# YamaguchiAtsushi/pointcloud_processor

Measured on AMD Instinct MI355X. Metric: ray-hit tests/sec + candidate poses/sec (whole node), 1M-pt terrain, higher is better.
Workload: dtype f64 march / f32 point test; 1 GPU; C2: 1M-pt L-shape excavation terrain, 1024x256 ray fan, 256 candidate poses per GPU; terrain_points=1001740, poses_total=256, num_candidates_lattice=348, parallelism=pose-shard x1

## Files before the change

pointcloud_processor_amd/_stamps.py:

```python
from __future__ import annotations

import hashlib
import os
from pathlib import Path

ROOT = Path(__file__).resolve().parents[1]
CSRC = ROOT / "pointcloud_processor_amd" / "csrc"
_COMMON = ["pcp_internal.hpp", "pcp_knobs.hpp", "Makefile", "../../include/pcp_abi.h"]
WORKLOAD_SOURCES = {
    "fan": ["pcp_fan.hip", "pcp_march.hpp", "pcp_fine.hip", "pcp_index.hip", "pcp_stencil.hpp",
            "pcp_grid.hpp", "pcp_fan_band.hpp", "pcp_fan_clear.hpp", "pcp_fan_clip.hpp",
            "pcp_fan_pivot.hpp", "pcp_fan_row.hpp"] + _COMMON,
    "filter": ["pcp_filter.hip", "pcp_rigid.hpp"] + _COMMON,
    "cells": ["pcp_score.hip", "pcp_march.hpp", "pcp_fine.hip", "pcp_index.hip", "pcp_stencil.hpp",
              "pcp_grid.hpp", "pcp_fan_band.hpp", "pcp_fan_clear.hpp", "pcp_fan_clip.hpp",
              "pcp_fan_pivot.hpp", "pcp_fan_row.hpp"] + _COMMON,
}


def workload_stamp(key: str) -> str:
    h = hashlib.sha256(os.environ.get("EXTRA", "").encode())
    for name in WORKLOAD_SOURCES[key]:
        f = (CSRC / name).resolve()
        h.update(name.encode())
        h.update(f.read_bytes())
    return h.hexdigest()[:16]
```

pointcloud_processor_amd/csrc/pcp_fan.hip:

```cpp
#pragma clang fp contract(off)

#include <algorithm>
#include <cmath>
#include <cstring>
#include <vector>

#include <hip/hip_ext.h>

#include "pcp_fan_cull.hpp"
#include "pcp_fan_dir.hpp"
#include "pcp_internal.hpp"
#include "pcp_march.hpp"

namespace pcp {

struct FanArgs {
    GridView g;
    const double *ca, *sa, *ce, *se;
    const double *pose;
    const double *steps;
    int K;
    int n_az;
    int uniform_el;
    uint32_t rays;
    uint32_t waves;
    float r2, rexit;
    int present;
    int16_t *first_hit;
    uint32_t w0, lw;
    int rev;
    uint2 *wave_part;
    uint32_t P;
    unsigned long long *stats;
};

enum { FAN_PLAIN = (int)FanMode::Plain, FAN_STATS = (int)FanMode::Stats,
       FAN_STAMPS = (int)FanMode::Stamps };

__device__ __forceinline__ uint32_t wave_sum_u32(uint32_t v) {
    v += (uint32_t)__builtin_amdgcn_update_dpp(0, (int)v, 0x128, 0xF, 0xF, false);
    v += (uint32_t)__builtin_amdgcn_update_dpp(0, (int)v, 0x124, 0xF, 0xF, false);
    v += (uint32_t)__builtin_amdgcn_update_dpp(0, (int)v, 0x122, 0xF, 0xF, false);
    v += (uint32_t)__builtin_amdgcn_update_dpp(0, (int)v, 0x121, 0xF, 0xF, false);
    return (uint32_t)__builtin_amdgcn_readlane((int)v, 0) +
           (uint32_t)__builtin_amdgcn_readlane((int)v, 16) +
           (uint32_t)__builtin_amdgcn_readlane((int)v, 32) +
           (uint32_t)__builtin_amdgcn_readlane((int)v, 48);
}

template <int MODE, int BS, bool ZB = true, int FN = 0, bool UE = false, int NPW = 1,
          bool SL = false, bool MT = false, bool SP = false>
__device__ __forceinline__ void fan_body(const FanArgs &a, uint32_t p0, uint32_t rblock) {
    static_assert(!MT || MODE == FAN_PLAIN, "the mounted march has no diagnostic modes");
    static_assert(!SP || !MT, "the mounted kernels keep the run-time layout tests");
    constexpr int PR = MT ? kFanDirRow : kFanRow;
    static_assert(PR * 32 * sizeof(double) + kStepLds * sizeof(double) <= 160 * 1024 / 8,
                  "at the widest NPW at least 8 one-wave workgroups per CU keep their LDS");
    const uint32_t ray = rblock * BS + threadIdx.x;
    const uint32_t wid = ray >> 6;
    const bool active = ray < a.rays;
    double lx = 0.0, ly = 0.0, lz = 0.0;
    __shared__ double s_steps[SL ? kStepLds : 1];
    __shared__ double s_pose[SL ? PR * NPW : 1];
    if (SL) {
        for (int q = threadIdx.x; q < a.K; q += BS) s_steps[q] = a.steps[q];
        for (int q = threadIdx.x; q < PR * NPW; q += BS) s_pose[q] = a.pose[PR * (size_t)p0 + q];
        __syncthreads();
    }
    const double *steps = SL ? s_steps : a.steps;
    uint32_t ju = 0;
    if (UE)
        ju = (uint32_t)__builtin_amdgcn_readfirstlane(
            (int)((rblock * BS + (threadIdx.x & ~63u)) / (uint32_t)a.n_az));
    if (active && a.present) {
        const uint32_t j = UE ? (rblock * BS + (threadIdx.x & ~63u)) / (uint32_t)a.n_az
                              : ray / (uint32_t)a.n_az;
        const uint32_t i = ray - j * (uint32_t)a.n_az;
        const double cej = a.ce[j];
        lx = cej * a.ca[i];
        ly = cej * a.sa[i];
        lz = a.se[j];
    }
#pragma unroll 1
    for (int q = 0; q < NPW; ++q) {
    const uint32_t p = p0 + (uint32_t)q;
    const uint32_t wslot = p * a.waves + wid;
    unsigned long long t0 = 0, t1 = 0, t2 = 0;
    if (MODE == FAN_STAMPS) t0 = __builtin_amdgcn_s_memtime();
    int hit = -1;
    uint32_t cnt[4] = {0, 0, 0, 0};
    const double *P = SL ? s_pose + PR * q : a.pose + PR * (size_t)p;
    bool dead = false;
    FanDir md{0.0, 0.0, 0.0};
    if (MT) md = fan_dir(P, lx, ly, lz);
    if (UE && !MT) {
        const uint2 lr = *reinterpret_cast<const uint2 *>(P + FR_LIVE);
        const uint32_t j0 = (uint32_t)__builtin_amdgcn_readfirstlane((int)lr.x);
        const uint32_t j1 = (uint32_t)__builtin_amdgcn_readfirstlane((int)lr.y);
        dead = ju < j0 || ju >= j1;
        if (MODE == FAN_STAMPS && dead) t1 = t0;
    }
    if (!dead && active && a.present) {
        const double cy = MT ? 0.0 : P[FR_CY], sy = MT ? 0.0 : P[FR_SY];
        const double dx = MT ? md.x : cy * lx - sy * ly;
        const double dy = MT ? md.y : sy * lx + cy * ly;
        const double dz = MT ? md.z : lz;
        if (MODE == FAN_STAMPS) {
            asm volatile("" ::"v"(dx), "v"(dy));
            t1 = __builtin_amdgcn_s_memtime();
        }
#ifdef PCP_FAN_NO_ROW
        constexpr bool ROW = false;
#else
        constexpr bool ROW = !MT;
#endif
        hit = march<MODE == FAN_STATS, ZB, 1, FN, true, true, ROW, SP>(
            a.g, P[0], P[1], P[2], dx, dy, dz, steps, a.K, 1e300, a.r2, a.rexit, cnt, 0, 1,
            MT ? nullptr : fan_row_floats(P));
    }
    if (MODE == FAN_STAMPS) {
        asm volatile("" ::"v"(hit));
        t2 = __builtin_amdgcn_s_memtime();
    }
    if (active && a.first_hit) a.first_hit[(size_t)p * a.rays + ray] = (int16_t)hit;
    uint2 part;
    if (UE && !MT && dead) {
        part = make_uint2(0u, 64u * (uint32_t)a.K);
    } else {
        const uint64_t bal = __ballot(active && hit >= 0);
        uint32_t u = active ? (hit >= 0 ? (uint32_t)hit + 1u : (uint32_t)a.K) : 0u;
        part = make_uint2((uint32_t)__popcll(bal), wave_sum_u32(u));
    }
    if ((threadIdx.x & 63) == 0 && wid < a.waves) {
        a.wave_part[(size_t)p * a.lw + (wid - a.w0)] = part;
    }
    if (MODE == FAN_STATS) {
        const size_t nw = (size_t)a.P * a.waves;
#pragma unroll
        for (int c = 0; c < 4; ++c) {
            unsigned long long v = c < 3 ? cnt[c] : (FN ? cnt[3] : cnt[1]);
#pragma unroll
            for (int o = 32; o > 0; o >>= 1) v += __shfl_xor(v, o, 64);
            if ((threadIdx.x & 63) == 0 && wid < a.waves) a.stats[c * nw + wslot] = v;
        }
    }
    if (MODE == FAN_STAMPS && (threadIdx.x & 63) == 0 && wid < a.waves) {
        const unsigned long long t3 = __builtin_amdgcn_s_memtime();
        unsigned long long *o = a.stats + 4 * (size_t)wslot;
        o[0] = t0;
        o[1] = t1;
        o[2] = t2;
        o[3] = t3;
    }
    }
}

template <int MODE, int BS = 64, bool ZB = true, int W = 7, int FN = 0, bool UE = false,
          bool MT = false>
__global__ void __launch_bounds__(BS) __attribute__((amdgpu_waves_per_eu(W, W)))
k_raycast_fan(FanArgs a, uint32_t P) {
    fan_body<MODE, BS, ZB, FN, UE, 1, false, MT>(a, blockIdx.x % P, a.w0 + blockIdx.x / P);
}

template <int MODE, int BS = 64, bool ZB = true, int W = 8, int FN = 1, bool UE = true, int NPW = 1,
          bool MT = false, bool SP = false>
__global__ void __launch_bounds__(BS) __attribute__((amdgpu_waves_per_eu(W, W)))
k_raycast_fan_xcd(FanArgs a, uint32_t P) {
    const uint32_t pc = P >> 3, gpc = pc / NPW, j = blockIdx.x >> 3;
    const uint32_t b = j / gpc;
    fan_body<MODE, BS, ZB, FN, UE, NPW, true, MT, SP>(a, (blockIdx.x & 7u) * pc + (j % gpc) * NPW,
                                                      a.w0 + (a.rev ? a.lw - 1u - b : b));
}

template <int BS, bool ZB>
__global__ void __launch_bounds__(BS) __attribute__((amdgpu_waves_per_eu(7, 7)))
k_raycast_fan_pm(FanArgs a, uint32_t) {
    fan_body<FAN_PLAIN, BS, ZB>(a, blockIdx.y, blockIdx.x);
}

__global__ void __launch_bounds__(1024)
k_sum_u64(const unsigned long long *__restrict__ in, size_t n, unsigned long long *__restrict__ out) {
    const unsigned long long *row = in + (size_t)blockIdx.x * n;
    unsigned long long v = 0;
    for (size_t k = threadIdx.x; k < n; k += 1024) v += row[k];
#pragma unroll
    for (int o = 32; o > 0; o >>= 1) v += __shfl_xor(v, o, 64);
    __shared__ unsigned long long sw[16];
    if ((threadIdx.x & 63) == 0) sw[threadIdx.x >> 6] = v;
    __syncthreads();
    if (threadIdx.x == 0) {
        unsigned long long t = 0;
        for (int w = 0; w < 16; ++w) t += sw[w];
        out[blockIdx.x] = t;
    }
}

__global__ void __launch_bounds__(kT)
k_fan_reduce(const uint2 *__restrict__ part, uint32_t waves,
             uint32_t *__restrict__ blocked, unsigned long long *__restrict__ units,
             unsigned long long *__restrict__ keys, uint32_t lo, uint32_t Pall,
             unsigned long long units_culled, int16_t *__restrict__ fh, uint32_t rays,
             uint32_t r_lo, uint32_t r_hi) {
    const uint32_t p = blockIdx.x;
    if (fh) {
        int16_t *row = fh + (size_t)p * rays;
        for (uint32_t r = threadIdx.x; r < r_lo; r += kT) row[r] = (int16_t)-1;
        for (uint32_t r = r_hi + threadIdx.x; r < rays; r += kT) row[r] = (int16_t)-1;
    }
    if (keys)
        for (uint32_t i = p * kT + threadIdx.x; i <= Pall; i += gridDim.x * kT)
            if (i < lo || i - lo >= gridDim.x) keys[i] = ~0ull;
    const uint2 *row = part + (size_t)p * waves;
    uint32_t b = 0;
    unsigned long long u = 0;
    for (uint32_t w = threadIdx.x; w < waves; w += kT) {
        const uint2 v = row[w];
        b += v.x;
        u += v.y;
    }
#pragma unroll
    for (int o = 32; o > 0; o >>= 1) {
        b += __shfl_xor(b, o, 64);
        u += __shfl_xor(u, o, 64);
    }
    __shared__ uint32_t sb[kT / 64];
    __shared__ unsigned long long su[kT / 64];
    if ((threadIdx.x & 63) == 0) {
// ... 430 lines not shown
```

pointcloud_processor_amd/csrc/pcp_fine.hip:

```cpp
#pragma clang fp contract(off)

#include <cfloat>
#include <cmath>

#include <rocprim/device/device_radix_sort.hpp>

#include "pcp_fan_band.hpp"
#include "pcp_fan_clear.hpp"
#include "pcp_fan_pivot.hpp"
#include "pcp_grid.hpp"
#include "pcp_internal.hpp"

namespace pcp {

namespace {

constexpr int kThreads = 256;

struct FineGeo {
    double ox, oy;
    double cf, inv_cf;
    double R2;
    int32_t fnx, fny;
    int32_t reach;
};

__device__ __forceinline__ bool in_window(const FineGeo &f, double px, double py, int wx, int wy) {
    const double x0 = f.ox + (double)wx * f.cf, y0 = f.oy + (double)wy * f.cf;
    const double dx = fmax(fmax(x0 - px, px - (x0 + f.cf)), 0.0);
    const double dy = fmax(fmax(y0 - py, py - (y0 + f.cf)), 0.0);
    return dx * dx + dy * dy <= f.R2;
}

__device__ __forceinline__ void fine_cell(const FineGeo &f, float x, float y, int &cx, int &cy) {
    cx = min(max((int)floor(((double)x - f.ox) * f.inv_cf), 0), f.fnx - 1);
    cy = min(max((int)floor(((double)y - f.oy) * f.inv_cf), 0), f.fny - 1);
}

__global__ void __launch_bounds__(kThreads)
k_zkeys(const float4 *__restrict__ pts, uint32_t n, unsigned long long *__restrict__ key,
        uint32_t *__restrict__ val) {
    const uint32_t i = blockIdx.x * kThreads + threadIdx.x;
    if (i >= n) return;
    const float4 p = pts[i];
    uint32_t u = __float_as_uint(p.z);
    u = (u & 0x80000000u) ? ~u : (u | 0x80000000u);
    key[i] = ((unsigned long long)(~u) << 32) | __float_as_uint(p.w);
    val[i] = i;
}

__global__ void __launch_bounds__(kThreads)
k_win_count(const float4 *__restrict__ pts, const uint32_t *__restrict__ zord, uint32_t n,
            FineGeo f, uint32_t *__restrict__ pcount) {
    const uint32_t i = blockIdx.x * kThreads + threadIdx.x;
    if (i >= n) return;
    const float4 p = pts[zord[i]];
    int cx, cy;
    fine_cell(f, p.x, p.y, cx, cy);
    uint32_t c = 0;
    for (int wy = max(cy - f.reach, 0); wy <= min(cy + f.reach, f.fny - 1); ++wy)
        for (int wx = max(cx - f.reach, 0); wx <= min(cx + f.reach, f.fnx - 1); ++wx)
            if (in_window(f, (double)p.x, (double)p.y, wx, wy)) ++c;
    pcount[i] = c;
}

__global__ void __launch_bounds__(kThreads)
k_win_emit(const float4 *__restrict__ pts, const uint32_t *__restrict__ zord, uint32_t n,
           FineGeo f, const uint32_t *__restrict__ poff, uint32_t *__restrict__ wkey,
           uint32_t *__restrict__ rank) {
    const uint32_t i = blockIdx.x * kThreads + threadIdx.x;
    if (i >= n) return;
    const float4 p = pts[zord[i]];
    int cx, cy;
    fine_cell(f, p.x, p.y, cx, cy);
    uint32_t o = poff[i];
    for (int wy = max(cy - f.reach, 0); wy <= min(cy + f.reach, f.fny - 1); ++wy)
        for (int wx = max(cx - f.reach, 0); wx <= min(cx + f.reach, f.fnx - 1); ++wx)
            if (in_window(f, (double)p.x, (double)p.y, wx, wy)) {
                wkey[o] = (uint32_t)wx + (uint32_t)f.fnx * (uint32_t)wy;
                rank[o] = i;
                ++o;
            }
}

__global__ void __launch_bounds__(kThreads)
k_win_bounds(const uint32_t *__restrict__ wkey, uint32_t np, uint32_t nw,
             uint32_t *__restrict__ cstart) {
    const uint32_t w = blockIdx.x * kThreads + threadIdx.x;
    if (w > nw) return;
    uint32_t lo = 0, hi = np;
    while (lo < hi) {
        const uint32_t mid = (lo + hi) >> 1;
        if (wkey[mid] < w) lo = mid + 1;
        else hi = mid;
    }
    cstart[w] = lo;
}

__global__ void __launch_bounds__(kThreads)
k_win_place(const float4 *__restrict__ pts, const uint32_t *__restrict__ zord,
            const uint32_t *__restrict__ wkey, const uint32_t *__restrict__ rank, uint32_t np,
            float4 *__restrict__ wpts) {
    const uint32_t k = blockIdx.x * kThreads + threadIdx.x;
    if (k >= np) return;
    wpts[k + wkey[k]] = pts[zord[rank[k]]];
}

__global__ void __launch_bounds__(kThreads)
k_frec(float4 *__restrict__ wpts, const uint32_t *__restrict__ cstart, CellMap m, double c,
       uint32_t fnx, uint32_t fny, uint32_t rz, uint32_t tsteps, int tile,
       int skip2, uint2 *__restrict__ frec, uint16_t *__restrict__ fband,
       uint32_t *__restrict__ fstart) {
    const uint32_t nw = fnx * fny, w = blockIdx.x * kThreads + threadIdx.x;
    const uint32_t sh = tile == 2 ? 3u : 2u, T = 1u << sh, TS = T * T;
    const uint32_t tx = (fnx + T - 1) >> sh, ty = (fny + T - 1) >> sh;
    const size_t plane = tile ? (size_t)tx * ty * TS : (size_t)nw;
    auto put = [&](size_t r, uint32_t start, uint32_t band) {
        if (tile == 2) {
            fband[r] = (uint16_t)band;
            fstart[r] = start;
        } else {
            frec[r] = make_uint2(start, band);
        }
    };
    if (tile && w < tx * ty * TS) {
        const uint32_t t = w >> (2 * sh), sub = w & (TS - 1);
        const uint32_t px = (t % tx) * T + (sub & (T - 1)), py = (t / tx) * T + (sub >> sh);
        if (px >= fnx || py >= fny)
            for (uint32_t iz = 0; iz < rz; ++iz) put((size_t)iz * plane + w, 0u, 0x00FFu);
    }
    if (w >= nw) return;
    const uint32_t wx = w % fnx, wy = w / fnx;
    const size_t base = tile ? ((size_t)((wy >> sh) * tx + (wx >> sh)) << (2 * sh)) |
                                   ((wy & (T - 1)) << sh) | (wx & (T - 1))
                             : (size_t)w;
    const uint32_t s = cstart[w] + w, e = cstart[w + 1] + w;
    wpts[e] = make_float4(__int_as_float(0x7FC00000), __int_as_float(0x7FC00000), -INFINITY,
                          __uint_as_float(0xFFFFFFFFu));
    uint32_t jt = s, jb = s, j2 = s, j3 = s;
    float zt = wpts[s].z, zb = zt, zlast = zt, z2 = zt, z3 = zt;
    int ct = s < e ? cell_z(m, zt) : -1, cb = ct;
    for (int iz = (int)rz - 1; iz >= 0; --iz) {
        while (jt < e && ct > iz + 1) {
            ++jt;
            zt = wpts[jt].z;
            ct = jt < e ? cell_z(m, zt) : -1;
        }
        if (jb < jt) {
            jb = jt;
            zb = zt;
            cb = ct;
        }
        while (jb < e && cb >= iz) {
            zlast = zb;
            ++jb;
            zb = wpts[jb].z;
            cb = jb < e ? cell_z(m, zb) : -1;
        }
        uint32_t band = 0x00FFu;
        if (jb > jt) {
            const uint32_t code = zband_code(zt, zlast, m.oz + (double)iz * c, c);
            const uint32_t lo = code & 255u, hi = code >> 8;
            const uint32_t lo2 = (lo == 0u || lo <= tsteps) ? 0u : lo - tsteps;
            const uint32_t hi2 = (hi == 255u) ? 255u : min(hi + tsteps, 255u);
// ... 113 lines not shown
}

__global__ void __launch_bounds__(kThreads)
k_pivot(const float4 *__restrict__ wpts, const uint32_t *__restrict__ cstart, FineGeo f,
        uint32_t tx, uint32_t nslot, float *__restrict__ piv) {
    const uint32_t t = blockIdx.x * kThreads + threadIdx.x;
    if (t >= nslot) return;
    const uint32_t tile = t >> 6, sub = t & 63u;
    const uint32_t wx = (tile % tx) * 8u + (sub & 7u), wy = (tile / tx) * 8u + (sub >> 3);
    float3 best = make_float3(__int_as_float(0x7FC00000), __int_as_float(0x7FC00000), -INFINITY);
    if (wx < (uint32_t)f.fnx && wy < (uint32_t)f.fny) {
        const uint32_t w = wx + (uint32_t)f.fnx * wy;
        const uint32_t s = cstart[w] + w, e = cstart[w + 1] + w;
        PivotKey kb{};
        for (uint32_t j = s; j < e; ++j) {
            const float4 p = wpts[j];
            const PivotKey k{pivot_d2(f.ox, f.oy, f.cf, wx, wy, p.x, p.y), p.z,
                             __float_as_uint(p.w)};
            if (j == s || pivot_better(k, kb)) {
                kb = k;
                best = make_float3(p.x, p.y, p.z);
            }
        }
    }
    float *o = piv + 3 * (size_t)t;
    o[0] = best.x;
    o[1] = best.y;
    o[2] = best.z;
}

__global__ void __launch_bounds__(kThreads)
k_pack3(const float4 *__restrict__ src, uint32_t n, float *__restrict__ dst) {
    const uint32_t i = blockIdx.x * kThreads + threadIdx.x;
    if (i >= n) return;
    const float4 p = src[i];
    dst[3 * (size_t)i] = p.x;
    dst[3 * (size_t)i + 1] = p.y;
    dst[3 * (size_t)i + 2] = p.z;
}

struct FinePlan {
    CellMap m;
    FineGeo f;
    ClearGeo cg;
    int F, tile;
    uint64_t fnx, fny, rz, nw, nrec;
    uint64_t npiv;
    size_t band_bytes, rec_bytes;
    uint32_t tsteps;
};

FinePlan fine_plan(const GridIndex &g, int F, int tile) {
    FinePlan p{};
    const GridView gv = g.view();
    p.m = CellMap{gv.ox, gv.oy, gv.oz, gv.inv_c, g.nx, g.ny, g.nz};
    p.F = F;
    p.tile = tile;
    p.fnx = (uint64_t)F * g.nx;
    p.fny = (uint64_t)F * g.ny;
    p.rz = (uint64_t)(g.nz > 1 ? g.nz - 1 : 0);
    const uint64_t T = tile == 2 ? 8 : 4;
    p.nrec = tile ? ((p.fnx + T - 1) / T) * ((p.fny + T - 1) / T) * T * T * p.rz
                  : p.fnx * p.fny * p.rz;
    p.nw = p.fnx * p.fny;
    p.npiv = tile == 2 ? (uint64_t)pivot_tiles((uint32_t)p.fnx) * pivot_tiles((uint32_t)p.fny) * 64
                       : 0;
    p.band_bytes = ((size_t)p.nrec * 2 + 255) & ~(size_t)255;
    p.rec_bytes = tile == 2 ? p.band_bytes + (size_t)p.nrec * 4 : (size_t)p.nrec * sizeof(uint2);
    p.f.ox = gv.ox;
    p.f.oy = gv.oy;
    p.f.cf = g.c / F;
    p.f.inv_cf = F * gv.inv_c;
    const double R = g.r_q + kQueryMargin;
    p.f.R2 = R * R;
    p.f.fnx = (int32_t)p.fnx;
    p.f.fny = (int32_t)p.fny;
    p.f.reach = (int32_t)std::ceil(R / p.f.cf);
    p.tsteps = (uint32_t)std::ceil((g.r_q + 2e-3) / g.c / (double)kZq);
    const double zabs = std::fmax(std::fabs(gv.oz), std::fabs(gv.oz + (double)g.nz * g.c));
    p.cg = fan_clear_geo(gv.oz, g.c, R, zabs);
    return p;
}

}

int build_fine(pcp_ctx *ctx, GridIndex &g) {
    if (g.fine_ok || g.fine_fail || !g.present || !g.occz_ok || g.n_pts == 0) return PCP_OK;
    hipStream_t st = ctx->stream;
    ProfScope prof(ctx, PCP_K_INDEX_BUILD);
    const FinePlan plan = fine_plan(g, std::max(2, std::min(ctx->knob.terrain_fine, 8)),
                                    ctx->knob.fine_tile == 2 ? 2 : ctx->knob.fine_tile ? 1 : 0);
    const CellMap m = plan.m;
    const FineGeo f = plan.f;
    const int F = plan.F, tile = plan.tile;
    const uint64_t fnx = plan.fnx, fny = plan.fny, rz = plan.rz, nrec = plan.nrec, nw = plan.nw;
    const size_t band_bytes = plan.band_bytes, rec_bytes = plan.rec_bytes;
    if (rz == 0 || nrec >= (1ull << 29) || fnx >= (1ull << 24) || fny * rz >= (1ull << 24)) {
        g.fine_fail = true;
        return PCP_OK;
    }
    const uint32_t n = (uint32_t)g.n_pts;
    const unsigned gridn = (n + kThreads - 1) / kThreads;
    const float4 *pts = g.pts.as<const float4>();
    size_t t1 = 0, t2 = 0;
    (void)rocprim::radix_sort_pairs(nullptr, t1, (unsigned long long *)nullptr,
                                    (unsigned long long *)nullptr, (uint32_t *)nullptr,
                                    (uint32_t *)nullptr, n, 0u, 64u, st);
    PCP_HIP(ctx, ctx->scratch[2].ensure((size_t)n * 24 + 64));
    unsigned long long *k0 = ctx->scratch[2].as<unsigned long long>(), *k1 = k0 + n;
    uint32_t *v0 = reinterpret_cast<uint32_t *>(k1 + n), *zord = v0 + n;
    hipLaunchKernelGGL(k_zkeys, dim3(gridn), dim3(kThreads), 0, st, pts, n, k0, v0);
    PCP_CHECK_LAUNCH(ctx);
    PCP_HIP(ctx, ctx->scratch[3].ensure((size_t)(n + 1) * 8 + (nw + 1) * 4 + 64));
    uint32_t *pcount = ctx->scratch[3].as<uint32_t>(), *poff = pcount + (n + 1);
    uint32_t *cstart = poff + (n + 1);
    const size_t tscan = scan_tmp_bytes(std::max<uint64_t>(n, nw)) +
                         (std::max<uint64_t>(n, nw) + 1) * sizeof(uint32_t);
    PCP_HIP(ctx, ctx->scratch[4].ensure(std::max(t1, tscan) + 256));
    if (rocprim::radix_sort_pairs(ctx->scratch[4].p, t1, k0, k1, v0, zord, n, 0u, 64u, st) !=
        hipSuccess)
        return set_err(ctx, PCP_E_HIP, "build_fine: z sort failed");
    hipLaunchKernelGGL(k_win_count, dim3(gridn), dim3(kThreads), 0, st, pts, zord, n, f, pcount);
    PCP_CHECK_LAUNCH(ctx);
    int rc = exclusive_scan_u32(ctx, pcount, poff, n, ctx->scratch[4].p);
    if (rc) return rc;
    uint32_t np = 0;
    if ((rc = read_small(ctx, &np, poff + n, 4, st))) return rc;
    if (np == 0 || (uint64_t)np + nw >= (1ull << 28)) {
        g.fine_fail = true;
        return PCP_OK;
    }
    int wbits = 1;
    while ((1ull << wbits) < nw) ++wbits;
    (void)rocprim::radix_sort_pairs(nullptr, t2, (uint32_t *)nullptr, (uint32_t *)nullptr,
                                    (uint32_t *)nullptr, (uint32_t *)nullptr, np, 0u,
                                    (unsigned)wbits, st);
    PCP_HIP(ctx, ctx->scratch[5].ensure((size_t)np * 16 + 64));
    uint32_t *wk0 = ctx->scratch[5].as<uint32_t>(), *wk1 = wk0 + np, *rk0 = wk1 + np,
             *rk1 = rk0 + np;
    PCP_HIP(ctx, ctx->scratch[6].ensure(t2 + 256));
    hipLaunchKernelGGL(k_win_emit, dim3(gridn), dim3(kThreads), 0, st, pts, zord, n, f,
                       (const uint32_t *)poff, wk0, rk0);
    PCP_CHECK_LAUNCH(ctx);
    if (rocprim::radix_sort_pairs(ctx->scratch[6].p, t2, wk0, wk1, rk0, rk1, np, 0u,
                                  (unsigned)wbits, st) != hipSuccess)
        return set_err(ctx, PCP_E_HIP, "build_fine: window sort failed");
    hipLaunchKernelGGL(k_win_bounds, dim3((unsigned)((nw + kThreads) / kThreads)), dim3(kThreads),
                       0, st, (const uint32_t *)wk1, np, (uint32_t)nw, cstart);
    PCP_CHECK_LAUNCH(ctx);
    const size_t nent = (size_t)np + nw;
    const bool pack = ctx->knob.fine_pack != 0;
    const bool pivots = tile == 2 && plan.npiv < (1ull << 28);
    if ((pack && ctx->scratch[7].ensure(nent * sizeof(float4)) != hipSuccess) ||
        g.wpts.ensure(pack ? nent * 12 + 16 : nent * sizeof(float4)) != hipSuccess ||
        g.frec.ensure(rec_bytes) != hipSuccess ||
        (pivots && g.fpiv.ensure(plan.npiv * kPivotBytes + 16) != hipSuccess)) {
        (void)hipGetLastError();
        g.wpts.release();
        g.frec.release();
        g.fpiv.release();
        g.fine_fail = true;
        return PCP_OK;
    }
    float4 *went = pack ? ctx->scratch[7].as<float4>() : g.wpts.as<float4>();
    hipLaunchKernelGGL(k_win_place, dim3((np + kThreads - 1) / kThreads), dim3(kThreads), 0, st,
                       pts, (const uint32_t *)zord, (const uint32_t *)wk1, (const uint32_t *)rk1,
                       np, went);
    PCP_CHECK_LAUNCH(ctx);
    const bool skip2 = tile == 2 && ctx->knob.fine_skip == 2 && nent < (1ull << 25);
    const uint32_t tsteps = plan.tsteps;
    const uint64_t nthr = std::max<uint64_t>(nw, tile ? nrec / rz : 0);
    hipLaunchKernelGGL(k_frec, dim3((unsigned)((nthr + kThreads - 1) / kThreads)), dim3(kThreads), 0,
                       st, went, (const uint32_t *)cstart, m, g.c, (uint32_t)fnx,
                       (uint32_t)fny, (uint32_t)rz, tsteps, tile, skip2 ? 1 : 0,
                       g.frec.as<uint2>(),
                       g.frec.as<uint16_t>(),
                       reinterpret_cast<uint32_t *>(g.frec.as<char>() + band_bytes));
    PCP_CHECK_LAUNCH(ctx);
    if (pivots) {
        hipLaunchKernelGGL(k_pivot, dim3((unsigned)((plan.npiv + kThreads - 1) / kThreads)),
                           dim3(kThreads), 0, st, (const float4 *)went, (const uint32_t *)cstart,
                           f, pivot_tiles((uint32_t)fnx), (uint32_t)plan.npiv,
                           g.fpiv.as<float>());
        PCP_CHECK_LAUNCH(ctx);
    }
    if (tile == 2) {
        const size_t lev_bytes = ((size_t)nw * 4 + 255) & ~(size_t)255;
        PCP_HIP(ctx, ctx->scratch[5].ensure(lev_bytes + (size_t)nw * rz * 2 + 64));
        uint32_t *lev = ctx->scratch[5].as<uint32_t>();
        uint16_t *hcol = reinterpret_cast<uint16_t *>(ctx->scratch[5].as<char>() + lev_bytes);
        const ClearGeo cg = plan.cg;
        PCP_HIP(ctx, hipMemsetAsync(lev, 0xFF, (size_t)nw * 4, st));
        hipLaunchKernelGGL(k_clear_level, dim3(gridn), dim3(kThreads), 0, st, pts, n, f, cg,
                           (int)rz, lev);
        PCP_CHECK_LAUNCH(ctx);
        const dim3 cgrid((unsigned)((nw + kThreads - 1) / kThreads), (unsigned)rz);
        hipLaunchKernelGGL(k_clear_col, dim3(cgrid.x), dim3(kThreads), 0, st,
                           (const uint32_t *)lev, (int)fnx, (int)fny, (uint32_t)nw, (uint32_t)rz,
                           hcol);
        PCP_CHECK_LAUNCH(ctx);
        hipLaunchKernelGGL(k_clear_code, cgrid, dim3(kThreads), 0, st, (const uint16_t *)hcol,
                           (int)fnx, (int)fny, (uint32_t)nw, (uint32_t)((fnx + 7) / 8), (size_t)(nrec / rz),
                           g.frec.as<uint16_t>());
        PCP_CHECK_LAUNCH(ctx);
        g.fband_ok = false;
        if (g.fband2.ensure(band_bytes) == hipSuccess) {
            PCP_HIP(ctx, hipMemcpyAsync(g.fband2.p, g.frec.p, band_bytes, hipMemcpyDeviceToDevice,
                                        st));
            hipLaunchKernelGGL(k_band_tight, dim3(cgrid.x), dim3(kThreads), 0, st,
                               (const float4 *)went, (const uint32_t *)cstart, m, f, g.c,
                               kQueryMargin, g.r_q + kBandMu, (uint32_t)rz,
                               (uint32_t)((fnx + 7) / 8), (size_t)(nrec / rz),
                               g.frec.as<const uint16_t>(), g.fband2.as<uint16_t>());
            PCP_CHECK_LAUNCH(ctx);
            g.fband_ok = true;
        } else {
            (void)hipGetLastError();
            g.fband2.release();
        }
    }
    if (pack) {
        hipLaunchKernelGGL(k_pack3, dim3((unsigned)((nent + kThreads - 1) / kThreads)),
                           dim3(kThreads), 0, st, (const float4 *)went, (uint32_t)nent,
                           g.wpts.as<float>());
        PCP_CHECK_LAUNCH(ctx);
    }
    g.wpack = pack ? 1 : 0;
    g.frx = (uint32_t)fnx;
    g.fry = (uint32_t)fny;
    g.frz = (uint32_t)rz;
    g.ffine = (float)F;
    g.ftile = tile;
    g.fskip = skip2 ? 2 : 1;
    g.fstart_off = tile == 2 ? band_bytes : 0;
    g.fnent = nent;
    g.fpiv_ok = pivots;
    g.fine_ok = true;
    return PCP_OK;
}

}

extern "C" int pcp_debug_fine_copy(pcp_ctx *ctx, pcp_fine_geo *geo, void *frec,
                                   uint64_t frec_cap, void *wpts, uint64_t wpts_cap, void *pts,
                                   uint64_t pts_cap) {
    using namespace pcp;
    if (!ctx || !geo) return PCP_E_INVALID;
    const GridIndex &g = ctx->terrain;
    *geo = pcp_fine_geo{};
    if (!g.present || !g.fine_ok) return PCP_OK;
    const FinePlan p = fine_plan(g, (int)g.ffine, g.ftile);
    geo->built = 1;
    geo->tile = g.ftile;
    geo->skip = g.fskip;
    geo->packed = g.wpack;
    geo->nx = g.nx;
    geo->ny = g.ny;
    geo->nz = g.nz;
    geo->F = p.F;
    geo->reach = p.f.reach;
    geo->fnx = p.f.fnx;
    geo->fny = p.f.fny;
    geo->rz = (int32_t)p.rz;
    geo->tsteps = (int32_t)p.tsteps;
    geo->n_points = g.n_pts;
    geo->n_records = p.nrec;
    geo->n_entries = g.fnent;
    geo->start_off = g.fstart_off;
    geo->frec_bytes = p.rec_bytes;
    geo->wpts_bytes = g.fnent * (g.wpack ? 12u : 16u);
    geo->pts_bytes = g.n_pts * sizeof(float4);
    geo->ox = p.m.ox;
    geo->oy = p.m.oy;
    geo->oz = p.m.oz;
    geo->c = g.c;
    geo->inv_c = p.m.inv_c;
    geo->r_q = g.r_q;
    geo->cf = p.f.cf;
    geo->inv_cf = p.f.inv_cf;
    geo->R2 = p.f.R2;
    geo->zq = (double)kZq;
    geo->clear_zt0 = p.cg.zt0;
    geo->clear_c = p.cg.c;
    if (!frec && !wpts && !pts) return PCP_OK;
    if ((frec && frec_cap < geo->frec_bytes) || (wpts && wpts_cap < geo->wpts_bytes) ||
        (pts && pts_cap < geo->pts_bytes))
        return set_err(ctx, PCP_E_CAPACITY, "pcp_debug_fine_copy: a buffer is too small");
    PCP_HIP(ctx, hipSetDevice(ctx->device));
    PCP_HIP(ctx, hipStreamSynchronize(ctx->stream));
    if (frec) PCP_HIP(ctx, hipMemcpy(frec, g.frec.p, geo->frec_bytes, hipMemcpyDeviceToHost));
    if (wpts) PCP_HIP(ctx, hipMemcpy(wpts, g.wpts.p, geo->wpts_bytes, hipMemcpyDeviceToHost));
    if (pts) PCP_HIP(ctx, hipMemcpy(pts, g.pts.p, geo->pts_bytes, hipMemcpyDeviceToHost));
    return PCP_OK;
}

extern "C" int pcp_debug_fine_pivot(pcp_ctx *ctx, pcp_fine_pivot_geo *geo, void *piv,
                                    uint64_t piv_cap) {
    using namespace pcp;
    if (!ctx || !geo) return PCP_E_INVALID;
    const GridIndex &g = ctx->terrain;
    *geo = pcp_fine_pivot_geo{};
    if (!g.present || !g.fine_ok || !g.fpiv_ok) return PCP_OK;
    const FinePlan p = fine_plan(g, (int)g.ffine, g.ftile);
    geo->built = 1;
    geo->enabled = ctx->knob.fan_pivot ? 1 : 0;
    geo->fnx = p.f.fnx;
    geo->fny = p.f.fny;
// ... 35 lines not shown
```

pointcloud_processor_amd/csrc/pcp_march.hpp:

```cpp
#pragma once

#include <cfloat>

#include "pcp_fan_clear.hpp"
#include "pcp_fan_clip.hpp"
#include "pcp_fan_row.hpp"
#include "pcp_internal.hpp"
#include "pcp_stencil.hpp"

namespace pcp {

constexpr int kT = 256;
#ifndef PCP_CELL_PROBES
#define PCP_CELL_PROBES 1
#endif

__device__ __forceinline__ bool stencil_cell(const GridView &g, float qx, float qy, float qz,
                                             uint32_t &lin) {
    uint32_t ix, iy, iz;
    const bool ok = stencil_cell3_fb(g, qx, qy, qz, ix, iy, iz);
    lin = ix + (uint32_t)g.nx * (iy + (uint32_t)g.ny * iz);
    return ok;
}

template <bool STATS>
__device__ __forceinline__ bool scan_stencil(const GridView &g, uint32_t lin, float qx, float qy,
                                             float qz, float r2, uint32_t *cnt) {
    const uint32_t nx = (uint32_t)g.nx, nxy = nx * (uint32_t)g.ny;
    uint32_t b[4][3];
#pragma unroll
    for (int r = 0; r < 4; ++r) {
        const U3 u = ld_u3o(g.start, lin + (r & 1) * nx + (r >> 1) * nxy);
        b[r][0] = u.a;
        b[r][1] = u.b;
        b[r][2] = u.c;
    }
    P3 f[8];
#pragma unroll
    for (int i = 0; i < 8; ++i) {
        const uint32_t k = b[i >> 1][i & 1];
        f[i] = ld_p3o(g.pts, k < b[i >> 1][(i & 1) + 1] ? k : 0u);
    }
    uint32_t live = 0;
#pragma unroll
    for (int i = 0; i < 8; ++i) {
        const uint32_t k = b[i >> 1][i & 1], e = b[i >> 1][(i & 1) + 1];
        if (k < e) {
            if (STATS) cnt[2] += 1;
            if (flann_within(qx, qy, qz, f[i], r2)) return true;
            const float dz = qz - f[i].z;
            if (!(dz >= 0.0f && dz * dz >= r2) && k + 1 < e) live |= 1u << i;
        }
    }
    if (!live) return false;
#pragma unroll
    for (int i = 0; i < 8; ++i) {
        if (!(live & (1u << i))) continue;
        const uint32_t e = b[i >> 1][(i & 1) + 1];
        for (uint32_t k = b[i >> 1][i & 1] + 1; k < e; k += 2) {
            const P3 p0 = ld_p3o(g.pts, k);
            const P3 p1 = ld_p3o(g.pts, min(k + 1, e - 1));
            if (STATS) cnt[2] += 1;
            if (flann_within(qx, qy, qz, p0, r2)) return true;
            float dz = qz - p0.z;
            if (dz >= 0.0f && dz * dz >= r2) break;
            if (k + 1 >= e) break;
            if (STATS) cnt[2] += 1;
            if (flann_within(qx, qy, qz, p1, r2)) return true;
            dz = qz - p1.z;
            if (dz >= 0.0f && dz * dz >= r2) break;
        }
    }
    return false;
}

#ifndef PCP_BLK_STEP
#define PCP_BLK_STEP 1
#endif
__device__ __forceinline__ uint32_t mad_u24(uint32_t a, uint32_t b, uint32_t c) {
    uint32_t d;
    asm("v_mad_u32_u24 %0, %1, %2, %3" : "=v"(d) : "v"(a), "v"(b), "v"(c));
    return d;
}
template <class T>
__device__ __forceinline__ T vgpr_pin(T x) {
#ifndef PCP_NO_VGPR_PIN
    asm("" : "+v"(x));
#endif
    return x;
}

template <bool STATS>
__device__ __forceinline__ bool scan_run(const float4 *pts, uint32_t k0, uint32_t e, float qx,
                                         float qy, float qz, float r2, uint32_t *cnt) {
    for (uint32_t k = k0; k < e; k += PCP_BLK_STEP) {
        P3 p[PCP_BLK_STEP];
#pragma unroll
        for (int i = 0; i < PCP_BLK_STEP; ++i) p[i] = ld_p3o(pts, min(k + i, e - 1));
#pragma unroll
        for (int i = 0; i < PCP_BLK_STEP; ++i) {
            if (i > 0 && k + i >= e) return false;
            if (STATS) cnt[2] += 1;
            if (flann_within(qx, qy, qz, p[i], r2)) return true;
            const float dz = qz - p[i].z;
            if (dz >= 0.0f && dz * dz >= r2) return false;
        }
    }
    return false;
}

template <bool STATS>
__device__ __forceinline__ bool scan_window3(const float *pts, uint32_t k, float qx, float qy,
                                             float qz, float r2, float rexit, uint32_t *cnt) {
    bool within, stop;
    do {
        const float *f = reinterpret_cast<const float *>(reinterpret_cast<const char *>(pts) +
                                                         ((k << 3) + (k << 2)));
        const P3 p = P3{f[0], f[1], f[2]};
        ++k;
        if (STATS) cnt[2] += 1;
#ifdef PCP_WALK_CENSUS
        if (STATS && p.z - qz >= rexit) cnt[3] += 1;
#endif
        within = flann_within(qx, qy, qz, p, r2);
        stop = within | (qz - p.z >= rexit);
    } while (!stop);
    return within;
}

template <bool STATS>
__device__ __forceinline__ bool scan_window(const float4 *pts, uint32_t k, float qx, float qy,
                                            float qz, float r2, float rexit, uint32_t *cnt) {
    bool within, stop;
    do {
        const P3 p = ld_p3o(pts, k++);
        if (STATS) cnt[2] += 1;
#ifdef PCP_WALK_CENSUS
        if (STATS && p.z - qz >= rexit) cnt[3] += 1;
#endif
        within = flann_within(qx, qy, qz, p, r2);
        stop = within | (qz - p.z >= rexit);
    } while (!stop);
    return within;
}

template <bool STATS>
__device__ __forceinline__ bool scan_block(const GridView &g, uint32_t lin, float qx, float qy,
                                           float qz, float r2, uint32_t *cnt) {
    const uint2 se = ld_u2o(g.bstart, lin);
    return scan_run<STATS>(g.bpts, se.x, se.y, qx, qy, qz, r2, cnt);
}

template <bool STATS>
__device__ __forceinline__ bool scan_corner(const GridView &g, uint32_t lin, float qx, float qy,
                                            float qz, float r2, uint32_t *cnt) {
    if (g.bpts) return scan_block<STATS>(g, lin, qx, qy, qz, r2, cnt);
    return scan_stencil<STATS>(g, lin, qx, qy, qz, r2, cnt);
}

__device__ __forceinline__ bool stencil_any(const GridView &g, float qx, float qy, float qz,
                                            float r2) {
    uint32_t lin;
    if (!stencil_cell(g, qx, qy, qz, lin)) return false;
    if (!((ld_u32o(g.occ2, lin >> 5) >> (lin & 31)) & 1u)) return false;
    return scan_stencil<false>(g, lin, qx, qy, qz, r2, nullptr);
}

__device__ __forceinline__ void clip_kf(const GridView &g, double px, double py, double pz,
                                        double dx, double dy, double dz, int K, int &klo,
                                        int &khi) {
    const float p[3] = {(float)px, (float)py, (float)pz};
    const float inv[3] = {__builtin_amdgcn_rcpf((float)dx), __builtin_amdgcn_rcpf((float)dy),
                          __builtin_amdgcn_rcpf((float)dz)};
    fan_clip(g.fb, p, inv, (float)(1.0 / kRayStep), g.fclip_e, K, klo, khi);
}
__device__ __forceinline__ void clip_kf_row(const GridView &g, const float *rel, double dx,
                                            double dy, double dz, int K, int &klo, int &khi) {
    const float inv[3] = {__builtin_amdgcn_rcpf((float)dx), __builtin_amdgcn_rcpf((float)dy),
                          __builtin_amdgcn_rcpf((float)dz)};
    fan_clip_rel(rel, inv, (float)(1.0 / kRayStep), g.fclip_e, K, klo, khi);
}

template <bool STATS, bool ZB = true, int NB = 1, int FN = 0, bool CLR = false, bool PIV = false,
          bool ROW = false, bool SP = false>
__device__ __forceinline__ int march(const GridView &g, double px, double py, double pz,
                                     double dx, double dy, double dz,
                                     const double *__restrict__ steps, int K, double end,
                                     float r2, float rexit, uint32_t *cnt = nullptr,
                                     int koff = 0, int kstr = 1, const float *rowf = nullptr) {
    static_assert(!SP || FN == 8, "the layout facts are the split records'");
    if (FN == 2) {
        if (g.frec && g.ftile == 2)
            return march<STATS, ZB, NB, 8, CLR, PIV, ROW>(g, px, py, pz, dx, dy, dz, steps, K,
                                                          end, r2, rexit, cnt, koff, kstr, rowf);
        if (g.frec && g.ftile)
            return march<STATS, ZB, NB, 4, CLR, PIV, ROW>(g, px, py, pz, dx, dy, dz, steps, K,
                                                          end, r2, rexit, cnt, koff, kstr, rowf);
        if (g.frec)
            return march<STATS, ZB, NB, 1, CLR, PIV, ROW>(g, px, py, pz, dx, dy, dz, steps, K,
                                                          end, r2, rexit, cnt, koff, kstr, rowf);
        return march<STATS, ZB, NB, 0, CLR, PIV, ROW>(g, px, py, pz, dx, dy, dz, steps, K, end,
                                                      r2, rexit, cnt, koff, kstr, rowf);
    }
    int klo, khi;
    if (ROW) clip_kf_row(g, rowf + FRF_CLIP, dx, dy, dz, K, klo, khi);
    else clip_kf(g, px, py, pz, dx, dy, dz, K, klo, khi);
    if (end < 1e299) {
        const double ke = floor((end - 0.5) / kRayStep) + 1.0;
        khi = (int)fmin((double)khi, fmax(ke, -1.0));
    }
    if (klo > khi) return -1;
    const float fdx = (float)dx, fdy = (float)dy, fdz = (float)dz;
    const float sc = (float)kRayStep * g.finv_c, h = 0.5f * g.finv_c;
    const float Dx = fdx * sc, Dy = fdy * sc, Dz = fdz * sc;
    const float Ax = (ROW ? rowf[FRF_BASE] : ((float)px - g.flo_x) * g.finv_c) + fdx * h;
    const float Ay = (ROW ? rowf[FRF_BASE + 1] : ((float)py - g.flo_y) * g.finv_c) + fdy * h;
    const float Az = (ROW ? rowf[FRF_BASE + 2] : ((float)pz - g.flo_z) * g.finv_c) + fdz * h;
    const uint32_t nx = (uint32_t)g.nx, ny = (uint32_t)g.ny;
    if (FN == 1 || FN == 4 || FN == 8) {
        const float F = g.ffine;
        const float D2x = F * Dx, D2y = F * Dy, A2x = F * (Ax + g.fzoff), A2y = F * (Ay + g.fzoff);
        const uint32_t mx = g.frx - 1, my = g.fry - 1, mz = g.frz - 1;
        const float fmx = (float)mx, fmy = (float)my, fmz = (float)mz;
        (void)mx, (void)my, (void)mz, (void)fmx, (void)fmy, (void)fmz;
        const uint32_t rxs = FN == 4 ? (g.frx + 3) >> 2 : FN == 8 ? (g.frx + 7) >> 3 : g.frx;
        const uint32_t rys = FN == 4 ? (g.fry + 3) >> 2 : FN == 8 ? (g.fry + 7) >> 3 : g.fry;
        const uint32_t rx = FN == 8 ? vgpr_pin(rxs) : rxs, ry = FN == 8 ? vgpr_pin(rys) : rys;
        const float fus_off = FN == 8 ? vgpr_pin(g.fus_off) : g.fus_off;
        const ClearRay cr = FN == 8 && CLR ? fan_clear_ray(fdx, fdy, fdz, (float)kRayStep, g.fclr_cf,
                                                    g.fclr_rb, SP || g.fclear != 0)
                                    : ClearRay{0.0f, 0.0f};
        for (int k = klo + koff, jump = 0; k <= khi; k += kstr * (1 + jump / kstr)) {
            const float kf = (float)k;
            const float fx = __builtin_fmaf(D2x, kf, A2x);
            const float fy = __builtin_fmaf(D2y, kf, A2y);
            const float fz = __builtin_fmaf(Dz, kf, Az);
#ifdef PCP_CLAMP_INT
            const uint32_t ix = min((uint32_t)fmaxf(fx, 0.0f), mx);
            const uint32_t iy = min((uint32_t)fmaxf(fy, 0.0f), my);
            const uint32_t iz = min((uint32_t)fmaxf(fz, 0.0f), mz);
#else
            const uint32_t ix = (uint32_t)__builtin_amdgcn_fmed3f(fx, 0.0f, fmx);
            const uint32_t iy = (uint32_t)__builtin_amdgcn_fmed3f(fy, 0.0f, fmy);
            const uint32_t iz = (uint32_t)__builtin_amdgcn_fmed3f(fz, 0.0f, fmz);
#endif
            const uint32_t ri = FN == 8 ? (mad_u24(rx, mad_u24(ry, iz, iy >> 3), ix >> 3) << 6) |
                                              ((iy & 7u) << 3) | (ix & 7u)
                              : FN == 4 ? (mad_u24(rx, mad_u24(ry, iz, iy >> 2), ix >> 2) << 4) |
                                              ((iy & 3u) << 2) | (ix & 3u)
                                        : mad_u24(rx, mad_u24(ry, iz, iy), ix);
            uint2 R = make_uint2(0u, 0u);
            if (FN == 8) R.y = ld_u16o(g.fband, ri);
            else R = ld_rec(g.frec, ri);
            const float us = __builtin_fmaf(fz - (float)iz, 1.0f / kZq, fus_off);
            const float lo = (float)(R.y & 255u);
            const bool cand = (us < (float)((R.y >> 8) & 255u)) & (us > lo);
            jump = (FN == 8 && CLR && lo == 255.0f) ? fan_clear_skip((float)(R.y >> 8), cr)
                                                    : 0;
            if (FN == 8 && CLR) asm volatile("" : "+v"(jump));
            if (STATS) cnt[0] += 1;
            if (cand) {
                const double s = steps[k];
                if (!(s < end)) return -1;
                const float qx = (float)(px + dx * s);
                const float qy = (float)(py + dy * s);
                const float qz = (float)(pz + dz * s);
                if (FN == 8 && PIV && (SP || g.fpiv)) {
                    const uint32_t pi = (mad_u24(rx, iy >> 3, ix >> 3) << 6) | (ri & 63u);
                    const float *pf = reinterpret_cast<const float *>(
                        reinterpret_cast<const char *>(g.fpiv) + ((pi << 3) + (pi << 2)));
                    const P3 pv = P3{pf[0], pf[1], pf[2]};
                    if (STATS) cnt[2] += 1;
                    if (flann_within(qx, qy, qz, pv, r2)) return k;
                }
                if (STATS) cnt[1] += 1;
                uint32_t w0 = R.x;
                if (FN == 8) {
                    const uint32_t ws = ld_u32o(g.fstart, ri);
                    if (SP || g.fskip == 2) {
                        const float ha = __builtin_fmaf((float)iz + 1.375f, g.fzc, g.fzo);
                        const float hb = __builtin_fmaf((float)iz + 1.6875f, g.fzc, g.fzo);
                        const float marg = 1e-4f + 4.0f * FLT_EPSILON *
                                                       (fmaxf(fabsf(ha), fabsf(hb)) +
                                                        fabsf(g.fzo) + fabsf(qz));
                        const float v = qz + (rexit + marg);
                        w0 = (ws & 0x01FFFFFFu) +
                             (v < ha ? (ws >> 25) & 15u : v < hb ? ws >> 29 : 0u);
                    } else {
                        const float h2 = __builtin_fmaf((float)iz + 1.5f, g.fzc, g.fzo);
                        const float marg =
                            1e-4f + 4.0f * FLT_EPSILON * (fabsf(h2) + fabsf(g.fzo) + fabsf(qz));
                        w0 = (ws & 0x0FFFFFFFu) + (qz + (rexit + marg) < h2 ? ws >> 28 : 0u);
                    }
                }
                const bool packed = SP || g.wpack;
                if (packed ? scan_window3<STATS>(reinterpret_cast<const float *>(g.wpts), w0, qx,
                                                 qy, qz, r2, rexit, cnt)
                           : scan_window<STATS>(g.wpts, w0, qx, qy, qz, r2, rexit, cnt))
                    return k;
            }
        }
        return -1;
    }
    if (NB > 1 && ZB) {
        for (int k0 = klo + NB * koff; k0 <= khi; k0 += NB * kstr) {
            uint32_t zz[NB], izs[NB];
            float fzs[NB];
#pragma unroll
            for (int b = 0; b < NB; ++b) {
                const float kf = (float)(k0 + b);
                const float fx = __builtin_fmaf(Dx, kf, Ax);
                const float fy = __builtin_fmaf(Dy, kf, Ay);
                const float fz = __builtin_fmaf(Dz, kf, Az);
                const bool ok = (k0 + b <= khi) & (fx >= 0.0f) & (fx < g.fnx1) & (fy >= 0.0f) &
                                (fy < g.fny1) & (fz >= 0.0f) & (fz < g.fnz1);
                const uint32_t izc = ok ? (uint32_t)fz : 0u;
                const uint32_t lin = ok ? (uint32_t)fx + nx * ((uint32_t)fy + ny * izc) : 0u;
                zz[b] = ok ? ld_u16o(g.occz, lin) : 0x00FFu;
                izs[b] = izc;
                fzs[b] = fz;
            }
#pragma unroll
            for (int b = 0; b < NB; ++b) {
                const int k = k0 + b;
                const uint32_t lo = zz[b] & 255u, hi = zz[b] >> 8;
                const float u = fzs[b] - (float)izs[b] + g.fzoff;
                const bool cand = (lo <= hi) & ((hi == 255u) | (u - (float)hi * kZq < g.fzt)) &
                                  ((lo == 0u) | ((float)lo * kZq - u < g.fzt));
                if (STATS && k <= khi) cnt[0] += 1;
                if (cand) {
                    const double s = steps[k];
                    if (!(s < end)) return -1;
                    if (STATS) cnt[1] += 1;
                    const float qx = (float)(px + dx * s);
                    const float qy = (float)(py + dy * s);
                    const float qz = (float)(pz + dz * s);
                    uint32_t l2;
                    if (stencil_cell(g, qx, qy, qz, l2) && scan_corner<STATS>(g, l2, qx, qy, qz, r2, cnt))
                        return k;
                }
            }
        }
        return -1;
    }
    for (int k = klo + koff; k <= khi; k += kstr) {
        const float kf = (float)k;
        const float fx = __builtin_fmaf(Dx, kf, Ax);
        const float fy = __builtin_fmaf(Dy, kf, Ay);
        const float fz = __builtin_fmaf(Dz, kf, Az);
        const bool ok = (fx >= 0.0f) & (fx < g.fnx1) & (fy >= 0.0f) & (fy < g.fny1) &
                        (fz >= 0.0f) & (fz < g.fnz1);
        const uint32_t izc = ok ? (uint32_t)fz : 0u;
        const uint32_t lin = ok ? (uint32_t)fx + nx * ((uint32_t)fy + ny * izc) : 0u;
        bool cand;
        if (ZB) {
            const uint32_t zz = ok ? ld_u16o(g.occz, lin) : 0x00FFu;
            const uint32_t lo = zz & 255u, hi = zz >> 8;
            const float u = fz - (float)izc + g.fzoff;
            cand = (lo <= hi) & ((hi == 255u) | (u - (float)hi * kZq < g.fzt)) &
                   ((lo == 0u) | ((float)lo * kZq - u < g.fzt));
        } else {
            const uint32_t word = ok ? ld_u32o(g.occ2, lin >> 5) : 0u;
            cand = (word >> (lin & 31u)) & 1u;
        }
        if (STATS) cnt[0] += 1;
        if (cand) {
            const double s = steps[k];
            if (!(s < end)) return -1;
            if (STATS) cnt[1] += 1;
            const float qx = (float)(px + dx * s);
            const float qy = (float)(py + dy * s);
            const float qz = (float)(pz + dz * s);
            uint32_t l2;
            if (stencil_cell(g, qx, qy, qz, l2) && scan_corner<STATS>(g, l2, qx, qy, qz, r2, cnt))
                return k;
        }
    }
    return -1;
}

}
```

Before: 8028 billion ray-hit tests/s.

## Pair-unroll packed window walk and hoist fan prologue loads before barrier

The packed 12-byte window scan now loads two consecutive entries per trip and tests them in order, so each iteration issues both loads up front instead of serialising one load per test. The allocation grows by a slack entry so the speculative second read stays in bounds. Separately, the shared-memory prologue now loads the step table, pose rows and trig values into registers before writing LDS and hitting the barrier, which lets all global loads overlap. The cost is extra loads on walks that stop after the first entry, plus more registers.

```diff
diff --git a/pointcloud_processor_amd/_stamps.py b/pointcloud_processor_amd/_stamps.py
--- a/pointcloud_processor_amd/_stamps.py
+++ b/pointcloud_processor_amd/_stamps.py
@@ -10,11 +10,11 @@
 WORKLOAD_SOURCES = {
     "fan": ["pcp_fan.hip", "pcp_march.hpp", "pcp_fine.hip", "pcp_index.hip", "pcp_stencil.hpp",
             "pcp_grid.hpp", "pcp_fan_band.hpp", "pcp_fan_clear.hpp", "pcp_fan_clip.hpp",
-            "pcp_fan_pivot.hpp", "pcp_fan_row.hpp"] + _COMMON,
+            "pcp_fan_pivot.hpp", "pcp_fan_row.hpp", "pcp_walk_pair.hpp"] + _COMMON,
     "filter": ["pcp_filter.hip", "pcp_rigid.hpp"] + _COMMON,
     "cells": ["pcp_score.hip", "pcp_march.hpp", "pcp_fine.hip", "pcp_index.hip", "pcp_stencil.hpp",
               "pcp_grid.hpp", "pcp_fan_band.hpp", "pcp_fan_clear.hpp", "pcp_fan_clip.hpp",
-              "pcp_fan_pivot.hpp", "pcp_fan_row.hpp"] + _COMMON,
+              "pcp_fan_pivot.hpp", "pcp_fan_row.hpp", "pcp_walk_pair.hpp"] + _COMMON,
 }
 
 
diff --git a/pointcloud_processor_amd/csrc/pcp_fan.hip b/pointcloud_processor_amd/csrc/pcp_fan.hip
--- a/pointcloud_processor_amd/csrc/pcp_fan.hip
+++ b/pointcloud_processor_amd/csrc/pcp_fan.hip
@@ -61,8 +61,46 @@
     const bool active = ray < a.rays;
     double lx = 0.0, ly = 0.0, lz = 0.0;
     __shared__ double s_steps[SL ? kStepLds : 1];
-    __shared__ double s_pose[SL ? PR * NPW : 1];
-    if (SL) {
+    __shared__ double s_pose[SL ? (PR * NPW + BS - 1) / BS * BS : 1];
+#ifdef PCP_FAN_NO_PRO1
+    constexpr bool PRO1 = false;
+#else
+    constexpr bool PRO1 = SL;
+#endif
+    if (PRO1) {
+        constexpr int NS = kStepLds / BS, NR = (PR * NPW + BS - 1) / BS;
+        static_assert(kStepLds % BS == 0, "whole trips over the step table");
+        double sv[NS], rv[NR], cej = 0.0, cai = 0.0, sai = 0.0, sej = 0.0;
+#pragma unroll
+        for (int t = 0; t < NS; ++t) {
+            const int q = (int)threadIdx.x + t * BS;
+            sv[t] = q < a.K ? a.steps[q] : 0.0;
+        }
+#pragma unroll
+        for (int t = 0; t < NR; ++t) {
+            const int q = (int)threadIdx.x + t * BS;
+            rv[t] = q < PR * NPW ? a.pose[PR * (size_t)p0 + q] : 0.0;
+        }
+        if (active && a.present) {
+            const uint32_t j = UE ? (rblock * BS + (threadIdx.x & ~63u)) / (uint32_t)a.n_az
+                                  : ray / (uint32_t)a.n_az;
+            const uint32_t i = ray - j * (uint32_t)a.n_az;
+            cej = a.ce[j];
+            cai = a.ca[i];
+            sai = a.sa[i];
+            sej = a.se[j];
+        }
+#pragma unroll
+        for (int t = 0; t < NS; ++t) s_steps[threadIdx.x + t * BS] = sv[t];
+#pragma unroll
+        for (int t = 0; t < NR; ++t) s_pose[threadIdx.x + t * BS] = rv[t];
+        __syncthreads();
+        if (active && a.present) {
+            lx = cej * cai;
+            ly = cej * sai;
+            lz = sej;
+        }
+    } else if (SL) {
         for (int q = threadIdx.x; q < a.K; q += BS) s_steps[q] = a.steps[q];
         for (int q = threadIdx.x; q < PR * NPW; q += BS) s_pose[q] = a.pose[PR * (size_t)p0 + q];
         __syncthreads();
@@ -72,7 +110,7 @@
     if (UE)
         ju = (uint32_t)__builtin_amdgcn_readfirstlane(
             (int)((rblock * BS + (threadIdx.x & ~63u)) / (uint32_t)a.n_az));
-    if (active && a.present) {
+    if (!PRO1 && active && a.present) {
         const uint32_t j = UE ? (rblock * BS + (threadIdx.x & ~63u)) / (uint32_t)a.n_az
                               : ray / (uint32_t)a.n_az;
         const uint32_t i = ray - j * (uint32_t)a.n_az;
diff --git a/pointcloud_processor_amd/csrc/pcp_fine.hip b/pointcloud_processor_amd/csrc/pcp_fine.hip
--- a/pointcloud_processor_amd/csrc/pcp_fine.hip
+++ b/pointcloud_processor_amd/csrc/pcp_fine.hip
@@ -10,6 +10,7 @@
 #include "pcp_fan_pivot.hpp"
 #include "pcp_grid.hpp"
 #include "pcp_internal.hpp"
+#include "pcp_walk_pair.hpp"
 
 namespace pcp {
 
@@ -429,7 +430,8 @@
     const bool pack = ctx->knob.fine_pack != 0;
     const bool pivots = tile == 2 && plan.npiv < (1ull << 28);
     if ((pack && ctx->scratch[7].ensure(nent * sizeof(float4)) != hipSuccess) ||
-        g.wpts.ensure(pack ? nent * 12 + 16 : nent * sizeof(float4)) != hipSuccess ||
+        g.wpts.ensure(pack ? nent * kWalkEntryBytes + kWalkPairSlack
+                           : nent * sizeof(float4)) != hipSuccess ||
         g.frec.ensure(rec_bytes) != hipSuccess ||
         (pivots && g.fpiv.ensure(plan.npiv * kPivotBytes + 16) != hipSuccess)) {
         (void)hipGetLastError();
diff --git a/pointcloud_processor_amd/csrc/pcp_march.hpp b/pointcloud_processor_amd/csrc/pcp_march.hpp
--- a/pointcloud_processor_amd/csrc/pcp_march.hpp
+++ b/pointcloud_processor_amd/csrc/pcp_march.hpp
@@ -7,6 +7,7 @@
 #include "pcp_fan_row.hpp"
 #include "pcp_internal.hpp"
 #include "pcp_stencil.hpp"
+#include "pcp_walk_pair.hpp"
 
 namespace pcp {
 
@@ -90,6 +91,12 @@
     return x;
 }
 
+#ifdef PCP_FAN_NO_PAIR
+template <bool SP> constexpr int kWalkSp = 1;
+#else
+template <bool SP> constexpr int kWalkSp = SP ? 2 : 1;
+#endif
+
 template <bool STATS>
 __device__ __forceinline__ bool scan_run(const float4 *pts, uint32_t k0, uint32_t e, float qx,
                                          float qy, float qz, float r2, uint32_t *cnt) {
@@ -109,22 +116,40 @@
     return false;
 }
 
-template <bool STATS>
+template <bool STATS, int WS = 1>
 __device__ __forceinline__ bool scan_window3(const float *pts, uint32_t k, float qx, float qy,
                                              float qz, float r2, float rexit, uint32_t *cnt) {
     bool within, stop;
+    if (WS == 2) {
+        do {
+            const float *f = walk_entry(pts, k);
+            const float ax = f[0], ay = f[1], az = f[2];
+            float bx = f[3], by = f[4], bz = f[5];
+            asm volatile("" : "+v"(bx), "+v"(by), "+v"(bz));
+            k += 2;
+            uint32_t t;
+            stop = walk_pair_step(ax, ay, az, bx, by, bz, qx, qy, qz, r2, rexit, within, t);
+            if (STATS) cnt[2] += t;
+        } while (!stop);
+        return within;
+    }
+    const uint32_t k0 = k;
+    (void)k0;
     do {
         const float *f = reinterpret_cast<const float *>(reinterpret_cast<const char *>(pts) +
                                                          ((k << 3) + (k << 2)));
         const P3 p = P3{f[0], f[1], f[2]};
         ++k;
         if (STATS) cnt[2] += 1;
-#ifdef PCP_WALK_CENSUS
+#if defined(PCP_WALK_CENSUS) && !defined(PCP_WALK_CENSUS_PAIR)
         if (STATS && p.z - qz >= rexit) cnt[3] += 1;
 #endif
         within = flann_within(qx, qy, qz, p, r2);
         stop = within | (qz - p.z >= rexit);
     } while (!stop);
+#if defined(PCP_WALK_CENSUS) && defined(PCP_WALK_CENSUS_PAIR)
+    if (STATS && ((k - k0) & 1u)) cnt[3] += 1;
+#endif
     return within;
 }
 
@@ -294,8 +319,9 @@
                     }
                 }
                 const bool packed = SP || g.wpack;
-                if (packed ? scan_window3<STATS>(reinterpret_cast<const float *>(g.wpts), w0, qx,
-                                                 qy, qz, r2, rexit, cnt)
+                if (packed ? scan_window3<STATS, kWalkSp<SP>>(
+                                 reinterpret_cast<const float *>(g.wpts), w0, qx, qy, qz, r2, rexit,
+                                 cnt)
                            : scan_window<STATS>(g.wpts, w0, qx, qy, qz, r2, rexit, cnt))
                     return k;
             }
diff --git a/pointcloud_processor_amd/csrc/pcp_walk_pair.hpp b/pointcloud_processor_amd/csrc/pcp_walk_pair.hpp
--- /dev/null
+++ b/pointcloud_processor_amd/csrc/pcp_walk_pair.hpp
@@ -0,0 +1,79 @@
+#pragma once
+
+#include <cstddef>
+#include <cstdint>
+
+#if defined(__HIPCC__)
+#define PCP_WP_HD __host__ __device__ __forceinline__
+#else
+#define PCP_WP_HD inline
+#endif
+
+namespace pcp {
+
+constexpr size_t kWalkEntryBytes = 12;
+constexpr int kWalkPairExtra = 1;
+constexpr size_t kWalkPairSlack = 16;
+static_assert(kWalkPairSlack >= kWalkPairExtra * kWalkEntryBytes, "an extra entry per trip");
+
+PCP_WP_HD bool walk_test(float px, float py, float pz, float qx, float qy, float qz, float r2,
+                         float rexit, bool &within) {
+    const float d0 = qx - px, d1 = qy - py, d2 = qz - pz;
+    float acc = 0.0f;
+    acc = acc + d0 * d0;
+    acc = acc + d1 * d1;
+    acc = acc + d2 * d2;
+    within = acc < r2;
+    return within | (qz - pz >= rexit);
+}
+
+PCP_WP_HD bool walk_pair_step(float ax, float ay, float az, float bx, float by, float bz,
+                              float qx, float qy, float qz, float r2, float rexit, bool &within,
+                              uint32_t &tests) {
+    tests = 1;
+    if (walk_test(ax, ay, az, qx, qy, qz, r2, rexit, within)) return true;
+    tests = 2;
+    return walk_test(bx, by, bz, qx, qy, qz, r2, rexit, within);
+}
+
+PCP_WP_HD const float *walk_entry(const float *pts, uint32_t k) {
+    return reinterpret_cast<const float *>(reinterpret_cast<const char *>(pts) +
+                                           ((k << 3) + (k << 2)));
+}
+
+struct WalkResult {
+    bool within;
+    uint32_t last;
+    uint32_t tests;
+};
+
+PCP_WP_HD WalkResult walk_single(const float *pts, uint32_t k, float qx, float qy, float qz,
+                                 float r2, float rexit) {
+    WalkResult w{false, k, 0};
+    bool stop;
+    do {
+        const float *f = walk_entry(pts, k);
+        w.last = k++;
+        w.tests += 1;
+        stop = walk_test(f[0], f[1], f[2], qx, qy, qz, r2, rexit, w.within);
+    } while (!stop);
+    return w;
+}
+
+PCP_WP_HD WalkResult walk_paired(const float *pts, uint32_t k, float qx, float qy, float qz,
+                                 float r2, float rexit) {
+    WalkResult w{false, k, 0};
+    bool stop;
+    do {
+        const float *f = walk_entry(pts, k);
+        const float ax = f[0], ay = f[1], az = f[2], bx = f[3], by = f[4], bz = f[5];
+        uint32_t t;
+        stop = walk_pair_step(ax, ay, az, bx, by, bz, qx, qy, qz, r2, rexit, w.within, t);
+        w.last = k + t - 1;
+        w.tests += t;
+        k += 2;
+    } while (!stop);
+    return w;
+}
+
+}
```

Result: faster. 8390 billion ray-hit tests/s, median of 6 (+4.5%).
